# ldyken53/gaussian-splatting-wgpu

Measured on AMD Instinct MI355X. Metric: frames/sec, higher is better.
Workload: dtype f32; 1 GPU; bicycle-like synthetic 6.1M gaussians @1920x1080; gaussians=6100000, width=1920, height=1080, tile_size=16, parallelism=single GPU, visible=2430918, processed=15909895, block_evaluated=6068168, sort_passes=1, depth_ordered_emission=True, tight_binning=True, blend_mode=fused, camera=64-step orbit, moved every frame

## Files before the change

### gaussian-splatting-wgpu_amd/csrc/gs_kernels.h

```cpp
#pragma once
#include "gs_device.h"

void gs_launch_repack(const void* d_aos, uint32_t n, const GsScene& s, hipStream_t st);
void gs_launch_ply_chunk(const void* d_raw, uint32_t m, uint32_t first, const GsPlyTable& t, const GsScene& s, hipStream_t st);
struct GsPreprocessLaunch {
    const void* func;
    uint32_t blocks;
    GsScene s; GsUniforms u; GsFrame f;
    void* gdata; uint32_t* counts; GsTightOut to;
    void* args[6];
};
void gs_preprocess_prepare(GsPreprocessLaunch& L, const GsScene& s, const GsUniforms& u, const GsFrame& f, void* gdata, uint32_t* counts,
                           bool tight, uint32_t* arena, uint32_t* rowptr, GsControl* ctl, uint32_t tight_nb = 0);
void gs_launch_preprocess(GsPreprocessLaunch& L, hipStream_t st);
void gs_launch_zero(void* p, uint64_t bytes, hipStream_t st);
uint32_t gs_scan_blocks(uint32_t n);
void gs_launch_scan(const uint32_t* counts, uint32_t n, uint32_t* offsets, unsigned long long* status, uint32_t* ticket, GsControl* ctl,
                    hipStream_t st);
uint64_t gs_emit_chunks(uint64_t capacity);
void gs_launch_emit_balanced(const void* gdata, const void* grec, const uint32_t* chunk_table, const GsFrame& f, uint32_t* keys, uint32_t* values,
                             GsControl* ctl, uint32_t grid, uint32_t hist_bits, uint32_t hist_passes, bool keys16, hipStream_t st);
void gs_launch_emit(const void* gdata, const uint32_t* counts, const uint32_t* offsets, const uint32_t* perm, const uint32_t* n_dev,
                    const GsFrame& f, uint32_t* keys, uint32_t* values, GsControl* ctl, hipStream_t st);
void gs_launch_ranges16(const uint16_t* tiles, const GsControl* ctl, uint32_t capacity, uint32_t T, uint32_t* ranges, uint32_t grid,
                        uint32_t* sticky, GsReport* rep, hipStream_t st);
void gs_launch_rebuild_keys(const uint16_t* tiles, const uint32_t* vals, const uint32_t* counts, uint32_t count, uint32_t n, uint32_t id_mask,
                            uint32_t* keys, hipStream_t st);
void gs_launch_ranges(const uint32_t* keys, const GsControl* ctl, uint32_t capacity, uint32_t T, uint32_t* ranges, uint32_t grid,
                      uint32_t* sticky, GsReport* rep, hipStream_t st);
uint32_t gs_sort_tiles(uint64_t capacity);
void gs_launch_sort(uint32_t* keysA, uint32_t* valsA, uint32_t* keysB, uint32_t* valsB, GsControl* ctl, uint32_t* tickets, uint32_t* hist,
                    const uint32_t* n_ptr, uint32_t capacity, uint32_t passes, uint32_t bits, uint32_t by_tile, uint32_t* status,
                    uint32_t grid, bool have_hist, const uint32_t* aux_table, uint32_t* aux_out, hipStream_t st, uint32_t** out_keys,
                    uint32_t** out_vals, bool keys16 = false);
int gs_launch_blend(const void* gdata, const uint32_t* values, const uint32_t* ranges, const GsFrame& f, uint32_t* rgba8, float* rgbf,
                    bool aux, float* alpha, float* depth, GsControl* ctl, uint32_t* tile_depth, bool exact, uint32_t ablation, bool masked, hipStream_t st, uint32_t* prof = nullptr,
                    uint32_t* prof_blocks = nullptr);
void gs_launch_debug_view(const uint32_t* ranges, const GsFrame& f, uint32_t view, uint32_t* rgba8, hipStream_t st);
void gs_launch_assemble(const void* slabs, void* image, uint32_t width, uint32_t height, const uint32_t* d_px_bounds, uint32_t n_slabs,
                        uint64_t slab_stride_px, hipStream_t st);
uint32_t gs_gsort_tiles(uint32_t n);
uint64_t gs_gsort_scratch_bytes(uint32_t n);
void gs_launch_gsort(const uint32_t* words, const uint32_t* aux_in, uint32_t n, void* scratch, void* grec, uint32_t* chunk_table, uint32_t chunk_cap,
                     uint32_t* tot_visible, uint32_t* tot_quantity, uint32_t grid, hipStream_t st);
uint32_t gs_rows_sort_tiles(uint64_t row_cap);
uint32_t gs_rows_chunks(uint64_t row_cap);
void gs_launch_rows(const uint32_t* arena, const void* grec, const uint32_t* chunk_table, uint32_t* rows_sorted, GsControl* ctl, uint32_t* sort_status, uint32_t row_cap,
                    uint32_t* M3, uint32_t* tileoff, uint32_t* rowtot, const GsFrame& f, uint32_t* values, uint32_t* ranges, uint32_t cus,
                    uint32_t* sticky, GsReport* rep, hipStream_t st, void (*mark)(void*, int), void* mark_arg);
void gs_launch_rows_rebuild_keys(const uint32_t* ranges, uint32_t T, const uint32_t* vals, const uint32_t* counts, uint32_t count, uint32_t n,
                                 uint32_t* keys, hipStream_t st);
void gs_launch_pick(const void* gdata, const uint32_t* values, const uint32_t* ranges, const GsFrame& f, uint32_t id_mask, const void* d_queries,
                    uint32_t n, void* d_results, uint32_t max_contrib, void* d_contrib, hipStream_t st);
```

### gaussian-splatting-wgpu_amd/csrc/gs_runtime.hip

```cpp
#include <hip/hip_runtime.h>

#include <algorithm>
#include <cmath>
#include <cstdarg>
#include <cstddef>
#include <cstdio>
#include <cstring>
#include <mutex>
#include <new>
#include <vector>

#include "../../include/gsplat/gs_abi.h"
#include "gs_kernels.h"
#include "gs_tight.h"

#define GS_EXPORT extern "C" __attribute__((visibility("default")))

static thread_local char g_err[512] = "";
static int32_t fail(int32_t code, const char* fmt, ...) {
    va_list ap;
    va_start(ap, fmt);
    vsnprintf(g_err, sizeof(g_err), fmt, ap);
    va_end(ap);
    return code;
}
#define HIP_TRY(expr)                                                                                       \
    do {                                                                                                    \
        hipError_t e_ = (expr);                                                                             \
        if (e_ != hipSuccess)                                                                               \
            return fail(e_ == hipErrorOutOfMemory ? GS_ERR_OUT_OF_MEMORY : GS_ERR_HIP, "%s: %s", #expr,      \
                        hipGetErrorString(e_));                                                             \
    } while (0)

#include <dlfcn.h>
namespace {
struct Roctx {
    int (*push)(const char*) = nullptr;
    int (*pop)() = nullptr;
    Roctx() {
// ... 9 lines not shown
Roctx& roctx() { static Roctx r; return r; }
const char* const kStageRange[] = {"gsplat:process_gaussians", "gsplat:exclusive_scan", "gsplat:write_tile_ids", "gsplat:radix_sort",
                                   "gsplat:compute_ranges", "gsplat:compute_tiles"};
}

#define GS_EV_RING 256
struct gs_ctx {
    gs_config cfg{};
    hipStream_t stream = nullptr;
    bool own_stream = false;
    GsFrame frame{};
    uint32_t T = 0, passes = 0, key_bits = 0;
    uint32_t tile_passes = 0, tile_bits = 0;
    bool tile16 = false;
    bool last_keys16 = false;
    uint32_t* keysG = nullptr;
    bool keysG_valid = false;
    int emit_order = 2;
    bool index_order = true;
    uint32_t debug_view = 0;
    uint32_t fif = 1;
    std::vector<gs_ctx*> shadows;
    bool is_shadow = false;
    gs_ctx* last = nullptr;
    uint32_t rr = 0;
    uint64_t cap_hint = 0, row_hint = 0;
    hipEvent_t ev_done = nullptr;
    uint64_t next_ticket = 1;
    struct { uint64_t ticket; gs_ctx* member; } tickets[64] = {};
    std::mutex ticket_mu;
    bool tile_cull = true;
    bool last_tight = false;
    uint32_t grid_persist = 0;
    uint32_t blend_ablation = 0;
    uint32_t* blend_prof = nullptr;
    uint32_t blend_prof_blocks = 0;
    void* scene_mem = nullptr;
    size_t scene_bytes = 0;
    GsScene scene{};
    uint32_t n = 0;
    uint32_t* counts = nullptr;
    uint32_t* offsets = nullptr;
    void* gdata = nullptr;
    uint64_t capacity = 0;
    uint32_t *keysA = nullptr, *valsA = nullptr, *keysB = nullptr, *valsB = nullptr;
    uint32_t *keysU = nullptr, *valsU = nullptr;
    uint32_t* chunk_table = nullptr;
    uint32_t *keysS = nullptr, *valsS = nullptr;
    void* ctl_mem = nullptr;
    size_t ctl_bytes = 0;
    GsControl* ctl = nullptr;
    unsigned long long* scan_status = nullptr;
    uint32_t* tile_depth = nullptr;
    uint32_t* sort_status = nullptr;
    uint32_t* rows_status = nullptr;
    void* grec = nullptr;
    uint32_t tight_nb = 0;
    void* gsort_scratch = nullptr;
    uint64_t row_cap = 0;
    uint32_t *arena = nullptr, *rows_sorted = nullptr, *rowptr = nullptr;
    uint32_t *M3 = nullptr, *tileoff = nullptr, *rowtot = nullptr;
    bool tight_ok = false;
    bool scene_borrowed = false;
    uint32_t last_passes = 0;
    bool last_by_index = true;
    uint32_t blend_walkers = 1;
// ... 105 lines not shown
    if (cfg->device < 0 || cfg->device >= ndev) return fail(GS_ERR_INVALID_ARGUMENT, "gs_create: device %d of %d", cfg->device, ndev);
    HIP_TRY(hipSetDevice(cfg->device));

    gs_ctx* c = new (std::nothrow) gs_ctx();
    if (!c) return fail(GS_ERR_OUT_OF_MEMORY, "gs_create: host allocation failed");
    c->cfg = *cfg;
    GsFrame& f = c->frame;
    f.width = cfg->width; f.height = cfg->height; f.tile_size = cfg->tile_size;
    f.ntx = tiles_f32(cfg->width, cfg->tile_size);
    f.nty = tiles_f32(cfg->height, cfg->tile_size);
    if (f.ntx >= 32768 || f.nty >= 65536) { delete c; return fail(GS_ERR_INVALID_ARGUMENT, "gs_create: canvas too large"); }
    f.col0 = cfg->col_begin;
    f.col1 = cfg->col_end;
    if (f.col0 == 0 && f.col1 == 0) f.col1 = f.ntx;
    if (f.col1 > f.ntx || f.col0 >= f.col1) { delete c; return fail(GS_ERR_INVALID_ARGUMENT, "gs_create: bad tile-column slab [%u,%u) of %u", f.col0, f.col1, f.ntx); }
    f.full = (f.col0 == 0 && f.col1 == f.ntx) ? 1u : 0u;
    f.px0 = f.col0 * f.tile_size;
    f.slab_w = std::min(f.width, f.col1 * f.tile_size) - f.px0;
    c->T = f.ntx * f.nty;
    const uint64_t max_key = ((uint64_t)f.nty * f.ntx + f.ntx) * 1000ull + 999ull;
    if (max_key > 0xFFFFFFFFull) { delete c; return fail(GS_ERR_INVALID_ARGUMENT, "gs_create: tile ids overflow the 32-bit key (write_tile_ids.wgsl:29)"); }
    c->key_bits = bits_for(max_key);
    c->passes = (c->key_bits + 7) / 8;
    const uint32_t tbits = bits_for((uint64_t)f.nty * f.ntx + f.ntx);
    c->tile_passes = (tbits + 7) / 8;
    c->tile_bits = (tbits + c->tile_passes - 1) / c->tile_passes;
    c->tile16 = ((uint64_t)f.nty * f.ntx + f.ntx) < 0xFFFFull;
    if ((uint64_t)(f.ntx + 1) * (f.nty + 1) > GS_COUNT_MASK) { delete c; return fail(GS_ERR_INVALID_ARGUMENT, "gs_create: canvas has too many tiles"); }
    c->tight_ok = f.ntx <= 255u && f.nty <= 255u;

    hipDeviceProp_t prop;
    HIP_TRY(hipGetDeviceProperties(&prop, cfg->device));
    c->grid_persist = (uint32_t)prop.multiProcessorCount * 4;
    if (cfg->stream) c->stream = (hipStream_t)cfg->stream;
    else { HIP_TRY(hipStreamCreateWithFlags(&c->stream, hipStreamNonBlocking)); c->own_stream = true; }

    HIP_TRY(hipMalloc((void**)&c->ranges, (size_t)c->T * 4));
    HIP_TRY(hipMemset(c->ranges, 0, (size_t)c->T * 4));
    const size_t px = (size_t)f.slab_w * f.height;
    HIP_TRY(hipMalloc((void**)&c->rgba8, px * 4));
    HIP_TRY(hipMemset(c->rgba8, 0, px * 4));
    if (cfg->flags & GS_FLAG_F32_TAP) HIP_TRY(hipMalloc((void**)&c->rgbf, px * 12));
    if (cfg->flags & GS_FLAG_AUX_OUTPUTS) {
        HIP_TRY(hipMalloc((void**)&c->alpha, px * 4));
        HIP_TRY(hipMalloc((void**)&c->depth, px * 4));
        HIP_TRY(hipMemset(c->alpha, 0, px * 4));
        HIP_TRY(hipMemset(c->depth, 0, px * 4));
    }
    HIP_TRY(hipHostMalloc((void**)&c->h_ctl, sizeof(GsControl), hipHostMallocDefault));
    memset(c->h_ctl, 0, sizeof(GsControl));
    HIP_TRY(hipMalloc((void**)&c->d_pxb, 65 * 4));
    HIP_TRY(hipMalloc((void**)&c->tileoff, 256 * 256 * 4));
    HIP_TRY(hipMalloc((void**)&c->rowtot, 256 * 4));
    HIP_TRY(hipMalloc((void**)&c->sticky, 4 * 4));
    HIP_TRY(hipMemset(c->sticky, 0, 4 * 4));
    HIP_TRY(hipHostMalloc((void**)&c->h_rep, sizeof(GsReport), hipHostMallocDefault));
    memset(c->h_rep, 0, sizeof(GsReport));
    if (cfg->flags & GS_FLAG_TIMING) {
        for (auto& row : c->ev)
            for (auto& e : row) HIP_TRY(hipEventCreate(&e));
        c->have_events = true;
    }
    c->fif = (c->own_stream && f.full) ? 3u : 1u;
    *out = c;
    return GS_OK;
}
// ... 128 lines not shown
    hipFree(d);
    return rc;
}

static inline void mark(gs_ctx* c, int i) {
    if (!c->have_events) return;
    hipEventRecord(c->ev[c->frames % GS_EV_RING][i], c->stream);
    Roctx& r = roctx();
    if (r.push) {
        if (i > 0) r.pop();
        if (i < GS_STAGE_COUNT) r.push(kStageRange[i]);
    }
}

static void mark_cb(void* p, int i) { mark((gs_ctx*)p, i); }

static int32_t record_frame(gs_ctx* c, const GsUniforms& u, bool debug, void* ext_rgba8, bool tight) {
    const GsFrame& f = c->frame;
    hipStream_t st = c->stream;
    gs_launch_zero(c->ctl_mem, tight ? c->ctl_bytes_tight : c->ctl_bytes, st);
    c->h_ctl_valid = false;
    if (debug) HIP_TRY(hipMemsetAsync(c->gdata, 0, std::max<size_t>((size_t)c->n * 64, 256), st));
    mark(c, 0);
    gs_preprocess_prepare(c->pre, c->scene, u, f, c->gdata, c->counts, tight, c->arena, c->rowptr, c->ctl, c->tight_nb);
    gs_launch_preprocess(c->pre, st);
    mark(c, 1);
    const bool by_index = !tight && (debug || c->index_order);
    bool keys16 = false;
    if (tight) {
        gs_launch_gsort(c->counts, c->rowptr, c->n, c->gsort_scratch, c->grec, c->chunk_table, (uint32_t)gs_emit_chunks(std::max(c->capacity, c->row_cap)),
                        &c->ctl->num_visible, &c->ctl->num_slots, c->grid_persist, st);
        mark(c, 2);
        gs_launch_rows(c->arena, c->grec, c->chunk_table, c->rows_sorted, c->ctl, c->rows_status, (uint32_t)c->row_cap, c->M3, c->tileoff, c->rowtot, f, c->valsA,
                       c->ranges, c->grid_persist / 4u, c->sticky, c->h_rep, st, mark_cb, c);
        c->keysS = nullptr;
        c->valsS = c->valsA;
        mark(c, 4);
    } else if (by_index) {
        gs_launch_scan(c->counts, c->n, c->offsets, c->scan_status, &c->ctl->scan_ticket[0], c->ctl, st);
        mark(c, 2);
        gs_launch_emit(c->gdata, c->counts, c->offsets, nullptr, nullptr, f, c->keysA, c->valsA, c->ctl, st);
    } else {
        gs_launch_gsort(c->counts, nullptr, c->n, c->gsort_scratch, c->grec, c->chunk_table, (uint32_t)gs_emit_chunks(std::max(c->capacity, c->row_cap)),
                        &c->ctl->num_visible, &c->ctl->num_intersections, c->grid_persist, st);
        mark(c, 2);
        gs_launch_emit_balanced(c->gdata, c->grec, c->chunk_table, f, c->keysA, c->valsA, c->ctl, c->grid_persist * 2,
                                c->tile_bits, c->tile_passes, c->tile16, st);
        keys16 = c->tile16;
    }
    if (debug) {
        if (!c->keysU) {
            HIP_TRY(hipMalloc((void**)&c->keysU, (size_t)c->capacity * 4));
            HIP_TRY(hipMalloc((void**)&c->valsU, (size_t)c->capacity * 4));
        }
        HIP_TRY(hipMemcpyAsync(c->keysU, c->keysA, (size_t)c->capacity * 4, hipMemcpyDeviceToDevice, st));
        HIP_TRY(hipMemcpyAsync(c->valsU, c->valsA, (size_t)c->capacity * 4, hipMemcpyDeviceToDevice, st));
    }
    if (!tight) {
        mark(c, 3);
        if (by_index)
            gs_launch_sort(c->keysA, c->valsA, c->keysB, c->valsB, c->ctl, c->ctl->sort_ticket, &c->ctl->hist[0][0], &c->ctl->num_intersections,
                           (uint32_t)c->capacity, c->passes, 8, 0, c->sort_status, c->grid_persist, false, nullptr, nullptr, st, &c->keysS, &c->valsS);
        else
            gs_launch_sort(c->keysA, c->valsA, c->keysB, c->valsB, c->ctl, c->ctl->sort_ticket, &c->ctl->hist[0][0], &c->ctl->num_intersections,
                           (uint32_t)c->capacity, c->tile_passes, c->tile_bits, keys16 ? 0 : 1, c->sort_status, c->grid_persist, true,
                           nullptr, nullptr, st, &c->keysS, &c->valsS, keys16);
        mark(c, 4);
// ... 156 lines not shown
}

static gs_ctx* last_of(gs_ctx* c) { return (c && c->last) ? c->last : c; }

GS_EXPORT int32_t gs_wait(gs_ctx* c) {
    if (!c) return fail(GS_ERR_INVALID_ARGUMENT, "gs_wait: null ctx");
    int32_t first = wait_one(c);
    char msg[sizeof(g_err)];
    if (first != GS_OK) memcpy(msg, g_err, sizeof(msg));
    for (gs_ctx* s : c->shadows) {
        const int32_t rc = wait_one(s);
        if (rc != GS_OK && first == GS_OK) { first = rc; memcpy(msg, g_err, sizeof(msg)); }
    }
    c->cap_hint = std::max(c->cap_hint, c->capacity);
    c->row_hint = std::max(c->row_hint, c->row_cap);
    for (gs_ctx* s : c->shadows) { c->cap_hint = std::max(c->cap_hint, s->capacity); c->row_hint = std::max(c->row_hint, s->row_cap); }
    if (first != GS_OK) memcpy(g_err, msg, sizeof(msg));
    return first;
}

static int32_t set_option_one(gs_ctx* c, int32_t key, int64_t value);
static int32_t add_shadow(gs_ctx* c) {
    gs_config cfg = c->cfg;
    cfg.stream = nullptr;
    cfg.max_intersections = 0;
    gs_ctx* s = nullptr;
    int32_t rc = gs_create(&cfg, &s);
    if (rc != GS_OK) return rc;
    s->fif = 1;
    s->is_shadow = true;
    rc = gs_share_splats(s, c);
    if (rc != GS_OK) { gs_destroy(s); return rc; }
    s->emit_order = c->emit_order; s->tile_cull = c->tile_cull; s->debug_view = c->debug_view;
    s->blend_ablation = c->blend_ablation; s->grid_persist = c->grid_persist; s->timed_from = 0; s->tight_nb = c->tight_nb;
    s->use_graph = c->use_graph;
    c->shadows.push_back(s);
    return GS_OK;
}

GS_EXPORT int32_t gs_render(gs_ctx* c, const void* uniforms) {
    if (!c || !uniforms) return fail(GS_ERR_INVALID_ARGUMENT, "gs_render: null argument");
    gs_ctx* t = c;
    if (c->fif > 1 && c->scene_mem) {
        if (c->pending && c->shadows.size() + 1 < c->fif) {
            int32_t rc = add_shadow(c);
            if (rc != GS_OK) return rc;
            c->rr = (uint32_t)c->shadows.size();
        }
        if (!c->shadows.empty()) {
            const uint32_t slot = c->rr++ % (uint32_t)(c->shadows.size() + 1);
            t = slot ? c->shadows[slot - 1] : c;
        }
        if (t->capacity < c->cap_hint || t->row_cap < c->row_hint) {
            HIP_TRY(hipSetDevice(t->cfg.device));
            if (t->pending) { int32_t rc = wait_one(t); if (rc != GS_OK && rc != GS_ERR_TRUNCATED) return rc; }
            hipFree(t->keysU); hipFree(t->valsU); t->keysU = t->valsU = nullptr;
            int32_t rc = alloc_kv(t, std::max(t->capacity, c->cap_hint), std::max(t->row_cap, c->row_hint));
            if (rc != GS_OK) return rc;
            t->have_frame = false;
        }
    }
    const int32_t rc = render_common(t, uniforms, false, nullptr);
    if (rc == GS_OK) c->last = t;
    return rc;
}
GS_EXPORT int32_t gs_render_host(gs_ctx* c, const void* uniforms, void* host_dst, uint64_t size, uint64_t* ticket) {
    if (!c || !uniforms || !host_dst || !ticket) return fail(GS_ERR_INVALID_ARGUMENT, "gs_render_host: null argument");
// ... 633 lines not shown
```

### gaussian-splatting-wgpu_amd/csrc/k_rows.hip

```cpp
#include "gs_device.h"
#include "gs_tight.h"

typedef uint32_t gs_item3 __attribute__((ext_vector_type(3), aligned(4)));

#ifndef RA_ITEMS
#define RA_ITEMS 8
#endif
#ifndef RA_WAVES
#define RA_WAVES 8
#endif
#define RA_THREADS (RA_WAVES * 64)
#define RA_TILE (RA_THREADS * RA_ITEMS)
#define RA_AGG (1u << 30)
#define RA_PREFIX (2u << 30)
#define RA_FLAGS (3u << 30)
#define RA_VALUE (~RA_FLAGS)

#ifndef RB_CH
#define RB_CH 512u
#endif
#define RB_IT (RB_CH / 256u)
#ifndef RB_SB
#define RB_SB 2048u
#endif
// ... 170 lines not shown
            const uint32_t r = (j & 1) ? (rank2[j >> 1] >> 16) : (rank2[j >> 1] & 0xFFFFu);
            const uint32_t pos = sh.hist[w][d] + r;
            sh.u.it[pos * 3 + 0] = ix[j];
            sh.u.it[pos * 3 + 1] = iy[j];
            sh.u.it[pos * 3 + 2] = iz[j];
        }
        __syncthreads();
        const uint32_t nvalid = sh.nvalid;
#pragma unroll
        for (int j = 0; j < RA_ITEMS; ++j) {
            const uint32_t pos = j * RA_THREADS + tid;
            if (pos < nvalid) {
                gs_item3 v;
                v.x = sh.u.it[pos * 3 + 0]; v.y = sh.u.it[pos * 3 + 1]; v.z = sh.u.it[pos * 3 + 2];
                const uint32_t g = sh.gbase[v.y & 0xFFu] + pos;
                if (g < row_cap) *reinterpret_cast<gs_item3*>(rows_out + (uint64_t)g * 3u) = v;
            }
        }
        __syncthreads();
    }
}

__device__ __forceinline__ unsigned long long wave_incl_scan64(unsigned long long v, uint32_t lane) {
#pragma unroll
    for (int d = 1; d < 64; d <<= 1) {
        const uint32_t lo = __shfl_up((uint32_t)v, d, 64), hi = __shfl_up((uint32_t)(v >> 32), d, 64);
        if ((int)lane >= d) v += ((unsigned long long)hi << 32) | lo;
    }
    return v;
}
struct RowTables {
    uint32_t ibase[257];
    uint32_t cbase[257];
    uint32_t w4[8];
};
__device__ __forceinline__ void row_tables(RowTables& T, const GsControl* ctl, uint32_t row_cap, uint32_t tid) {
    const uint32_t lane = tid & 63, w = tid >> 6;
    const bool on = tid < 256u;
    const uint32_t c = on ? gs_rowhist(ctl, tid) : 0u;
    const unsigned long long ic = wave_incl_scan64(c, lane);
    if (on && lane == 63) { T.w4[w] = (uint32_t)(ic > 0xFFFFFFFFull ? 0xFFFFFFFFull : ic); }
    __syncthreads();
    uint32_t i0 = 0, cc = 0;
    if (on) {
        unsigned long long b = ic - c;
        for (uint32_t k = 0; k < w; ++k) b += T.w4[k];
        const unsigned long long e = b + c;
        i0 = b > row_cap ? row_cap : (uint32_t)b;
        const uint32_t i1 = e > row_cap ? row_cap : (uint32_t)e;
        cc = i1 - i0;
        T.ibase[tid] = i0;
        if (tid == 255u) T.ibase[256] = i1;
    }
    const uint32_t ch = (cc + RB_CH - 1u) / RB_CH;
    const uint32_t ih = wave_incl_scan(ch, lane);
    if (on && lane == 63) T.w4[4 + w] = ih;
    __syncthreads();
    if (on) {
        uint32_t bh = 0;
        for (uint32_t k = 0; k < w; ++k) bh += T.w4[4 + k];
        T.cbase[tid] = bh + ih - ch;
        if (tid == 255u) T.cbase[256] = bh + ih;
    }
    __syncthreads();
}
__device__ __forceinline__ uint32_t row_of_chunk(const RowTables& T, uint32_t c) {
    const uint32_t lane = threadIdx.x & 63u;
    uint32_t v[4];
#pragma unroll
    for (int k = 0; k < 4; ++k) v[k] = T.cbase[lane + 64u * k];
    uint32_t r = 0;
#pragma unroll
    for (int k = 0; k < 4; ++k) r += (uint32_t)__popcll(__ballot(v[k] <= c && (lane + 64u * k) != 0u));
    return r;
}

__global__ __launch_bounds__(256) void gs_rows_count_kernel(const uint32_t* __restrict__ rows, const GsControl* ctl, uint32_t* __restrict__ M3,
                                                            uint32_t chunk_cap, uint32_t row_cap) {
    __shared__ RowTables T;
    __shared__ int s_diff[257];
    __shared__ uint32_t s_w[4];
    const uint32_t tid = threadIdx.x, lane = tid & 63, w = tid >> 6;
    row_tables(T, ctl, row_cap, tid);
    uint32_t nch = T.cbase[256];
    if (nch > chunk_cap) nch = chunk_cap;
    for (uint32_t c = blockIdx.x; c < nch; c += gridDim.x) {
        const uint32_t r = row_of_chunk(T, c);
        const uint32_t i0 = T.ibase[r] + (c - T.cbase[r]) * RB_CH;
        const uint32_t i1 = (i0 + RB_CH < T.ibase[r + 1]) ? i0 + RB_CH : T.ibase[r + 1];
        s_diff[tid] = 0;
        if (tid == 0) s_diff[256] = 0;
        __syncthreads();
#pragma unroll
        for (int k = 0; k < (int)(RB_CH / 256u); ++k) {
            const uint32_t i = i0 + k * 256u + tid;
            if (i < i1) {
                const uint32_t w1 = rows[(uint64_t)i * 3u + 1u];
                const uint32_t tlo = (w1 >> 8) & 0xFFu, len = ((w1 >> 16) & 0xFFu) + 1u;
                atomicAdd(&s_diff[tlo], 1);
                atomicAdd(&s_diff[tlo + len > 256u ? 256u : tlo + len], -1);
            }
        }
        __syncthreads();
        const uint32_t v = (uint32_t)s_diff[tid];
        const uint32_t incl = wave_incl_scan(v, lane);
        if (lane == 63) s_w[w] = incl;
        __syncthreads();
        uint32_t b = 0;
        for (uint32_t k = 0; k < w; ++k) b += s_w[k];
        M3[(uint64_t)c * 256u + tid] = b + incl;
        __syncthreads();
    }
}

__global__ __launch_bounds__(1024) void gs_rows_scan_kernel(const GsControl* ctl, uint32_t* __restrict__ M3, uint32_t* __restrict__ tileoff,
                                                            uint32_t* __restrict__ rowtot, uint32_t chunk_cap, uint32_t row_cap) {
    __shared__ RowTables T;
    __shared__ unsigned long long s_part[4][256];
    __shared__ unsigned long long s_ex[256];
    __shared__ unsigned long long s_w[4];
    const uint32_t tid = threadIdx.x, c = tid & 255u, p = tid >> 8, r = blockIdx.x;
    row_tables(T, ctl, row_cap, tid);
    uint32_t c0 = T.cbase[r], c1 = T.cbase[r + 1];
    if (c0 > chunk_cap) c0 = chunk_cap;
    if (c1 > chunk_cap) c1 = chunk_cap;
    const uint32_t nch = c1 - c0, per = (nch + 3u) / 4u;
    const uint32_t j0 = c0 + (p * per < nch ? p * per : nch), j1 = c0 + ((p + 1u) * per < nch ? (p + 1u) * per : nch);
    unsigned long long sum = 0;
    for (uint32_t j = j0; j < j1; j += 8u) {
        uint32_t v[8];
#pragma unroll
        for (int k = 0; k < 8; ++k) v[k] = (j + k < j1) ? M3[(uint64_t)(j + k) * 256u + c] : 0u;
#pragma unroll
        for (int k = 0; k < 8; ++k) sum += v[k];
    }
    s_part[p][c] = sum;
    __syncthreads();
    unsigned long long run = 0, tot = 0;
#pragma unroll
    for (int k = 0; k < 4; ++k) { const unsigned long long t = s_part[k][c]; if (k < (int)p) run += t; tot += t; }
    for (uint32_t j = j0; j < j1; j += 8u) {
        uint32_t v[8];
#pragma unroll
        for (int k = 0; k < 8; ++k) v[k] = (j + k < j1) ? M3[(uint64_t)(j + k) * 256u + c] : 0u;
#pragma unroll
        for (int k = 0; k < 8; ++k) {
            if (j + k < j1) M3[(uint64_t)(j + k) * 256u + c] = run > 0xFFFFFFFFull ? 0xFFFFFFFFu : (uint32_t)run;
            run += v[k];
        }
    }
    if (p == 0) {
        const uint32_t lane = tid & 63, w = tid >> 6;
        unsigned long long incl = tot;
#pragma unroll
        for (int d = 1; d < 64; d <<= 1) {
            const uint32_t lo = __shfl_up((uint32_t)incl, d, 64), hi = __shfl_up((uint32_t)(incl >> 32), d, 64);
// ... 2 lines not shown
        if (lane == 63) s_w[w] = incl;
        s_ex[c] = incl - tot;
    }
    __syncthreads();
    if (p == 0) {
        const uint32_t w = tid >> 6;
        unsigned long long b = 0, all = 0;
#pragma unroll
        for (int k = 0; k < 4; ++k) { if (k < (int)w) b += s_w[k]; all += s_w[k]; }
        const unsigned long long ex = b + s_ex[c];
        tileoff[r * 256u + c] = ex > 0xFFFFFFFFull ? 0xFFFFFFFFu : (uint32_t)ex;
        if (c == 0) rowtot[r] = all > 0xFFFFFFFFull ? 0xFFFFFFFFu : (uint32_t)all;
    }
}

struct ExpandShared {
    RowTables T;
    uint32_t rbase[257];
    uint32_t w0[RB_CH], w1[RB_CH], w2[RB_CH];
    uint32_t hist[4][256];
    uint32_t gbase[256];
    uint32_t wsum[8];
    uint32_t nvalid, total;
    unsigned char cols[RB_SB];
    union {
        struct { uint32_t P[RB_CH + 1]; unsigned short mark[RB_SB]; } e;
        uint32_t vals[RB_SB];
    } x;
};

__global__ __launch_bounds__(256) void gs_rows_expand_kernel(const uint32_t* __restrict__ rows, GsControl* ctl, const uint32_t* __restrict__ M3,
                                                             const uint32_t* __restrict__ tileoff, const uint32_t* __restrict__ rowtot, GsFrame f,
                                                             uint32_t* __restrict__ values, uint32_t* __restrict__ ranges, uint32_t chunk_cap,
                                                             uint32_t row_cap, uint32_t* sticky, GsReport* rep) {
    __shared__ ExpandShared S;
    const uint32_t tid = threadIdx.x, lane = tid & 63, w = tid >> 6;
    const unsigned long long lt_mask = (1ull << lane) - 1ull;
    const uint32_t ns = f.tile_size >= 16u ? 2u : 1u;
    const uint32_t hole = f.ntx < 128u ? 127u : 255u;
    const int nbits = f.ntx < 128u ? 7 : 8;
    row_tables(S.T, ctl, row_cap, tid);
    {
        const uint32_t v = tid < f.nty ? rowtot[tid] : 0u;
        unsigned long long incl = v;
#pragma unroll
        for (int d = 1; d < 64; d <<= 1) {
            const uint32_t lo = __shfl_up((uint32_t)incl, d, 64), hi = __shfl_up((uint32_t)(incl >> 32), d, 64);
            if ((int)lane >= d) incl += ((unsigned long long)hi << 32) | lo;
        }
        __shared__ unsigned long long s_r[4];
        if (lane == 63) s_r[w] = incl;
        __syncthreads();
        unsigned long long b = 0;
        for (uint32_t k = 0; k < w; ++k) b += s_r[k];
        const unsigned long long ex = b + incl - v;
        S.rbase[tid] = ex > 0xFFFFFFFFull ? 0xFFFFFFFFu : (uint32_t)ex;
        if (tid == 255u) S.rbase[256] = (b + incl) > 0xFFFFFFFFull ? 0xFFFFFFFFu : (uint32_t)(b + incl);
        __syncthreads();
    }
    if (blockIdx.x == 0 && tid == 0) {
        const uint32_t I = S.rbase[256];
        ctl->num_intersections = I;
        ctl->num_items = S.T.ibase[256];
        if (I > f.capacity) ctl->overflow = 1u;
        gs_frame_report(ctl, I, S.T.ibase[256], f.capacity, sticky, rep);
    }
    for (uint32_t r = blockIdx.x; r < f.nty; r += gridDim.x) {
        if (tid < f.ntx) {
            const uint32_t endoff = (tid + 1u < 256u) ? tileoff[r * 256u + tid + 1u] : rowtot[r];
            const unsigned long long e = (unsigned long long)S.rbase[r] + endoff;
            ranges[r * f.ntx + tid] = e > 0xFFFFFFFFull ? 0xFFFFFFFFu : (uint32_t)e;
        }
    }
    uint32_t nch = S.T.cbase[256];
    if (nch > chunk_cap) nch = chunk_cap;
    gs_item3 nit[RB_IT];
    uint32_t n_r = 0, n_ni = 0, n_tstart = 0, n_done = 0;
    auto prefetch = [&](uint32_t c) {
        n_r = row_of_chunk(S.T, c);
        const uint32_t i0 = S.T.ibase[n_r] + (c - S.T.cbase[n_r]) * RB_CH;
        const uint32_t i1 = (i0 + RB_CH < S.T.ibase[n_r + 1]) ? i0 + RB_CH : S.T.ibase[n_r + 1];
        n_ni = i1 - i0;
#pragma unroll
        for (int k = 0; k < (int)RB_IT; ++k) {
            const uint32_t e = tid * RB_IT + k;
            nit[k] = *reinterpret_cast<const gs_item3*>(rows + (uint64_t)(i0 + (e < n_ni ? e : 0u)) * 3u);
        }
        n_tstart = S.rbase[n_r] + tileoff[n_r * 256u + tid];
        n_done = M3[(uint64_t)c * 256u + tid];
    };
    if (blockIdx.x < nch) prefetch(blockIdx.x);
    for (uint32_t c = blockIdx.x; c < nch; c += gridDim.x) {
        const uint32_t ni = n_ni;
        uint32_t len[RB_IT], lsum = 0;
#pragma unroll
        for (int k = 0; k < (int)RB_IT; ++k) {
            const uint32_t e = tid * RB_IT + k;
            len[k] = 0u;
            if (e < ni) {
                S.w0[e] = nit[k].x; S.w1[e] = nit[k].y; S.w2[e] = nit[k].z;
                len[k] = ((nit[k].y >> 16) & 0xFFu) + 1u;
            }
            lsum += len[k];
        }
        const uint32_t tstart = n_tstart;
        uint32_t done = n_done;
        if (c + gridDim.x < nch) prefetch(c + gridDim.x);
        {
            const uint32_t incl = wave_incl_scan(lsum, lane);
            if (lane == 63) S.wsum[w] = incl;
            __syncthreads();
            uint32_t b = 0, all = 0;
#pragma unroll
            for (int k = 0; k < 4; ++k) { if (k < (int)w) b += S.wsum[k]; all += S.wsum[k]; }
            uint32_t run = b + incl - lsum;
#pragma unroll
            for (int k = 0; k < (int)RB_IT; ++k) { S.x.e.P[tid * RB_IT + k] = run; run += len[k]; }
            if (tid == 0) { S.x.e.P[RB_CH] = all; S.total = all; }
        }
        __syncthreads();
        const uint32_t ninst = S.total;
        for (uint32_t s0 = 0; s0 < ninst; s0 += RB_SB) {
            if (s0) {
                __syncthreads();
                uint32_t l2[RB_IT], ls = 0;
#pragma unroll
                for (int k = 0; k < (int)RB_IT; ++k) { const uint32_t e = tid * RB_IT + k; l2[k] = e < ni ? ((S.w1[e] >> 16) & 0xFFu) + 1u : 0u; ls += l2[k]; }
                const uint32_t incl = wave_incl_scan(ls, lane);
                if (lane == 63) S.wsum[w] = incl;
                __syncthreads();
                uint32_t b = 0;
#pragma unroll
                for (int k = 0; k < 4; ++k) if (k < (int)w) b += S.wsum[k];
                uint32_t run = b + incl - ls;
#pragma unroll
                for (int k = 0; k < (int)RB_IT; ++k) { S.x.e.P[tid * RB_IT + k] = run; run += l2[k]; }
                if (tid == 0) S.x.e.P[RB_CH] = ninst;
            }
            for (uint32_t k = tid; k < RB_SB / 2u; k += 256u) reinterpret_cast<uint32_t*>(S.x.e.mark)[k] = 0u;
            for (uint32_t k = lane; k < 256; k += 64) S.hist[w][k] = 0u;
// ... 102 lines not shown
#pragma unroll
            for (int j = 0; j < (int)RB_PER; ++j) {
                const uint32_t pos = j * 256u + tid;
                if (pos < nvalid) {
                    const uint32_t dst = S.gbase[S.cols[pos]] + pos;
                    if (dst < f.capacity) values[dst] = S.x.vals[pos];
                }
            }
        }
        __syncthreads();
    }
}

__global__ __launch_bounds__(256) void gs_rows_rebuild_keys_kernel(const uint32_t* __restrict__ ranges, uint32_t T, const uint32_t* __restrict__ vals,
                                                                   const uint32_t* __restrict__ counts, uint32_t count, uint32_t n,
                                                                   uint32_t* __restrict__ keys) {
    for (uint32_t i = blockIdx.x * 256u + threadIdx.x; i < count; i += gridDim.x * 256u) {
        uint32_t lo = 0, hi = T;
        while (lo < hi) {
            const uint32_t mid = (lo + hi) >> 1;
            if (ranges[mid] > i) hi = mid; else lo = mid + 1u;
        }
        const uint32_t g = vals[i] & GS_ID_MASK;
        keys[i] = lo * 1000u + (g < n ? counts[g] >> GS_COUNT_BITS : 0u);
    }
}

#ifndef RB_CNT_WG
#define RB_CNT_WG 8u
#endif
#ifndef RB_EXP_WG
#define RB_EXP_WG 6u
#endif
uint32_t gs_rows_sort_tiles(uint64_t row_cap) { return (uint32_t)((row_cap + RA_TILE - 1) / RA_TILE); }
uint32_t gs_rows_chunks(uint64_t row_cap) { return (uint32_t)(row_cap / RB_CH + 256u); }
void gs_launch_rows(const uint32_t* arena, const void* grec, const uint32_t* chunk_table, uint32_t* rows_sorted, GsControl* ctl, uint32_t* sort_status, uint32_t row_cap,
                    uint32_t* M3, uint32_t* tileoff, uint32_t* rowtot, const GsFrame& f, uint32_t* values, uint32_t* ranges, uint32_t cus,
                    uint32_t* sticky, GsReport* rep, hipStream_t st, void (*mark)(void*, int), void* mark_arg) {
    const uint32_t chunk_cap = gs_rows_chunks(row_cap);
    if (!cus) cus = 1;
    hipLaunchKernelGGL(gs_rows_sort_kernel, dim3(cus * 3u), dim3(RA_THREADS), 0, st, arena, (const uint4*)grec, chunk_table, rows_sorted, ctl, sort_status,
                       row_cap, f.nty);
    if (mark) mark(mark_arg, 3);
    hipLaunchKernelGGL(gs_rows_count_kernel, dim3(cus * RB_CNT_WG), dim3(256), 0, st, (const uint32_t*)rows_sorted, (const GsControl*)ctl, M3, chunk_cap, row_cap);
    hipLaunchKernelGGL(gs_rows_scan_kernel, dim3(f.nty), dim3(1024), 0, st, (const GsControl*)ctl, M3, tileoff, rowtot, chunk_cap, row_cap);
    hipLaunchKernelGGL(gs_rows_expand_kernel, dim3(cus * RB_EXP_WG), dim3(256), 0, st, (const uint32_t*)rows_sorted, ctl, (const uint32_t*)M3,
                       (const uint32_t*)tileoff, (const uint32_t*)rowtot, f, values, ranges, chunk_cap, row_cap, sticky, rep);
}
void gs_launch_rows_rebuild_keys(const uint32_t* ranges, uint32_t T, const uint32_t* vals, const uint32_t* counts, uint32_t count, uint32_t n,
                                 uint32_t* keys, hipStream_t st) {
    if (!count) return;
    const uint32_t blocks = (count + 255u) / 256u;
    hipLaunchKernelGGL(gs_rows_rebuild_keys_kernel, dim3(blocks < 4096u ? blocks : 4096u), dim3(256), 0, st, ranges, T, vals, counts, count, n, keys);
}
```

Baseline: 1378 frames/s.

## Group row chunks into multi-chunk runs for count/scan/expand

Adds a run abstraction in the rows binning pipeline: consecutive chunks within a row are grouped into runs of K chunks, sized so the total run count is close to a target (by default a multiple of the expand grid). The count kernel now builds one histogram per run, so M3 stores per-run prefix counts. The scan works over runs and the expand kernel walks K chunks of a run in sequence, reloading tile start and done counts only at run heads. The aim is fewer M3 entries, less scan work and fewer per-chunk global reads. The cost is coarser load balance and longer serial work per block.

Result: no change. 1391 frames/s, median of 6 (+1.0%).

```diff
diff --git a/gaussian-splatting-wgpu_amd/csrc/gs_kernels.h b/gaussian-splatting-wgpu_amd/csrc/gs_kernels.h
--- a/gaussian-splatting-wgpu_amd/csrc/gs_kernels.h
+++ b/gaussian-splatting-wgpu_amd/csrc/gs_kernels.h
@@ -47,7 +47,7 @@
 uint32_t gs_rows_chunks(uint64_t row_cap);
 void gs_launch_rows(const uint32_t* arena, const void* grec, const uint32_t* chunk_table, uint32_t* rows_sorted, GsControl* ctl, uint32_t* sort_status, uint32_t row_cap,
                     uint32_t* M3, uint32_t* tileoff, uint32_t* rowtot, const GsFrame& f, uint32_t* values, uint32_t* ranges, uint32_t cus,
-                    uint32_t* sticky, GsReport* rep, hipStream_t st, void (*mark)(void*, int), void* mark_arg);
+                    uint32_t runs, uint32_t* sticky, GsReport* rep, hipStream_t st, void (*mark)(void*, int), void* mark_arg);
 void gs_launch_rows_rebuild_keys(const uint32_t* ranges, uint32_t T, const uint32_t* vals, const uint32_t* counts, uint32_t count, uint32_t n,
                                  uint32_t* keys, hipStream_t st);
 void gs_launch_pick(const void* gdata, const uint32_t* values, const uint32_t* ranges, const GsFrame& f, uint32_t id_mask, const void* d_queries,
diff --git a/gaussian-splatting-wgpu_amd/csrc/gs_runtime.hip b/gaussian-splatting-wgpu_amd/csrc/gs_runtime.hip
--- a/gaussian-splatting-wgpu_amd/csrc/gs_runtime.hip
+++ b/gaussian-splatting-wgpu_amd/csrc/gs_runtime.hip
@@ -5,6 +5,7 @@
 #include <cstdarg>
 #include <cstddef>
 #include <cstdio>
+#include <cstdlib>
 #include <cstring>
 #include <mutex>
 #include <new>
@@ -80,6 +81,7 @@
     bool tile_cull = true;
     bool last_tight = false;
     uint32_t grid_persist = 0;
+    uint32_t rows_runs = 0;
     uint32_t blend_ablation = 0;
     uint32_t* blend_prof = nullptr;
     uint32_t blend_prof_blocks = 0;
@@ -251,6 +253,10 @@
     hipDeviceProp_t prop;
     HIP_TRY(hipGetDeviceProperties(&prop, cfg->device));
     c->grid_persist = (uint32_t)prop.multiProcessorCount * 4;
+    if (const char* e = getenv("GSPLAT_ROWS_RUNS")) {
+        const unsigned long long v = strtoull(e, nullptr, 10);
+        c->rows_runs = v > 0x7FFFFFFFull ? 0x7FFFFFFFu : (uint32_t)v;
+    }
     if (cfg->stream) c->stream = (hipStream_t)cfg->stream;
     else { HIP_TRY(hipStreamCreateWithFlags(&c->stream, hipStreamNonBlocking)); c->own_stream = true; }
 
@@ -445,7 +451,7 @@
                         &c->ctl->num_visible, &c->ctl->num_slots, c->grid_persist, st);
         mark(c, 2);
         gs_launch_rows(c->arena, c->grec, c->chunk_table, c->rows_sorted, c->ctl, c->rows_status, (uint32_t)c->row_cap, c->M3, c->tileoff, c->rowtot, f, c->valsA,
-                       c->ranges, c->grid_persist / 4u, c->sticky, c->h_rep, st, mark_cb, c);
+                       c->ranges, c->grid_persist / 4u, c->rows_runs, c->sticky, c->h_rep, st, mark_cb, c);
         c->keysS = nullptr;
         c->valsS = c->valsA;
         mark(c, 4);
@@ -668,7 +674,7 @@
     rc = gs_share_splats(s, c);
     if (rc != GS_OK) { gs_destroy(s); return rc; }
     s->emit_order = c->emit_order; s->tile_cull = c->tile_cull; s->debug_view = c->debug_view;
-    s->blend_ablation = c->blend_ablation; s->grid_persist = c->grid_persist; s->timed_from = 0; s->tight_nb = c->tight_nb;
+    s->blend_ablation = c->blend_ablation; s->grid_persist = c->grid_persist; s->rows_runs = c->rows_runs; s->timed_from = 0; s->tight_nb = c->tight_nb;
     s->use_graph = c->use_graph;
     c->shadows.push_back(s);
     return GS_OK;
diff --git a/gaussian-splatting-wgpu_amd/csrc/k_rows.hip b/gaussian-splatting-wgpu_amd/csrc/k_rows.hip
--- a/gaussian-splatting-wgpu_amd/csrc/k_rows.hip
+++ b/gaussian-splatting-wgpu_amd/csrc/k_rows.hip
@@ -226,9 +226,11 @@
 struct RowTables {
     uint32_t ibase[257];
     uint32_t cbase[257];
+    uint32_t ubase[257];
+    uint32_t K;
     uint32_t w4[8];
 };
-__device__ __forceinline__ void row_tables(RowTables& T, const GsControl* ctl, uint32_t row_cap, uint32_t tid) {
+__device__ __forceinline__ void row_tables(RowTables& T, const GsControl* ctl, uint32_t row_cap, uint32_t G, uint32_t tid) {
     const uint32_t lane = tid & 63, w = tid >> 6;
     const bool on = tid < 256u;
     const uint32_t c = on ? gs_rowhist(ctl, tid) : 0u;
@@ -257,6 +259,20 @@
         if (tid == 255u) T.cbase[256] = bh + ih;
     }
     __syncthreads();
+    const uint32_t nch = T.cbase[256], g = G ? G : 1u;
+    uint32_t K = nch / g + (nch % g ? 1u : 0u);
+    if (K < 1u) K = 1u;
+    const uint32_t ru = ch / K + (ch % K ? 1u : 0u);
+    const uint32_t iu = wave_incl_scan(ru, lane);
+    if (on && lane == 63) T.w4[w] = iu;
+    __syncthreads();
+    if (on) {
+        uint32_t bu = 0;
+        for (uint32_t k = 0; k < w; ++k) bu += T.w4[k];
+        T.ubase[tid] = bu + iu - ru;
+        if (tid == 255u) { T.ubase[256] = bu + iu; T.K = K; }
+    }
+    __syncthreads();
 }
 __device__ __forceinline__ uint32_t row_of_chunk(const RowTables& T, uint32_t c) {
     const uint32_t lane = threadIdx.x & 63u;
@@ -268,31 +284,49 @@
     for (int k = 0; k < 4; ++k) r += (uint32_t)__popcll(__ballot(v[k] <= c && (lane + 64u * k) != 0u));
     return r;
 }
+__device__ __forceinline__ uint32_t row_of_run(const RowTables& T, uint32_t u) {
+    const uint32_t lane = threadIdx.x & 63u;
+    uint32_t v[4];
+#pragma unroll
+    for (int k = 0; k < 4; ++k) v[k] = T.ubase[lane + 64u * k];
+    uint32_t r = 0;
+#pragma unroll
+    for (int k = 0; k < 4; ++k) r += (uint32_t)__popcll(__ballot(v[k] <= u && (lane + 64u * k) != 0u));
+    return r;
+}
 
 __global__ __launch_bounds__(256) void gs_rows_count_kernel(const uint32_t* __restrict__ rows, const GsControl* ctl, uint32_t* __restrict__ M3,
-                                                            uint32_t chunk_cap, uint32_t row_cap) {
+                                                            uint32_t chunk_cap, uint32_t row_cap, uint32_t G) {
     __shared__ RowTables T;
     __shared__ int s_diff[257];
     __shared__ uint32_t s_w[4];
     const uint32_t tid = threadIdx.x, lane = tid & 63, w = tid >> 6;
-    row_tables(T, ctl, row_cap, tid);
-    uint32_t nch = T.cbase[256];
-    if (nch > chunk_cap) nch = chunk_cap;
-    for (uint32_t c = blockIdx.x; c < nch; c += gridDim.x) {
-        const uint32_t r = row_of_chunk(T, c);
-        const uint32_t i0 = T.ibase[r] + (c - T.cbase[r]) * RB_CH;
-        const uint32_t i1 = (i0 + RB_CH < T.ibase[r + 1]) ? i0 + RB_CH : T.ibase[r + 1];
+    row_tables(T, ctl, row_cap, G, tid);
+    uint32_t nrun = T.ubase[256];
+    if (nrun > chunk_cap) nrun = chunk_cap;
+    const uint32_t K = T.K;
+    for (uint32_t u = blockIdx.x; u < nrun; u += gridDim.x) {
+        const uint32_t r = row_of_run(T, u);
+        const uint32_t i0 = T.ibase[r] + (u - T.ubase[r]) * K * RB_CH;
+        const uint32_t left = T.ibase[r + 1] - i0;
+        const uint32_t ni = (unsigned long long)K * RB_CH < left ? K * RB_CH : left;
         s_diff[tid] = 0;
         if (tid == 0) s_diff[256] = 0;
         __syncthreads();
-#pragma unroll
-        for (int k = 0; k < (int)(RB_CH / 256u); ++k) {
-            const uint32_t i = i0 + k * 256u + tid;
-            if (i < i1) {
-                const uint32_t w1 = rows[(uint64_t)i * 3u + 1u];
-                const uint32_t tlo = (w1 >> 8) & 0xFFu, len = ((w1 >> 16) & 0xFFu) + 1u;
-                atomicAdd(&s_diff[tlo], 1);
-                atomicAdd(&s_diff[tlo + len > 256u ? 256u : tlo + len], -1);
+        for (uint32_t o = 0; o < ni; o += 4u * 256u) {
+            uint32_t w1[4];
+#pragma unroll
+            for (int k = 0; k < 4; ++k) {
+                const uint32_t i = o + k * 256u + tid;
+                w1[k] = rows[(uint64_t)(i0 + (i < ni ? i : 0u)) * 3u + 1u];
+            }
+#pragma unroll
+            for (int k = 0; k < 4; ++k) {
+                if (o + k * 256u + tid < ni) {
+                    const uint32_t tlo = (w1[k] >> 8) & 0xFFu, len = ((w1[k] >> 16) & 0xFFu) + 1u;
+                    atomicAdd(&s_diff[tlo], 1);
+                    atomicAdd(&s_diff[tlo + len > 256u ? 256u : tlo + len], -1);
+                }
             }
         }
         __syncthreads();
@@ -302,20 +336,20 @@
         __syncthreads();
         uint32_t b = 0;
         for (uint32_t k = 0; k < w; ++k) b += s_w[k];
-        M3[(uint64_t)c * 256u + tid] = b + incl;
+        M3[(uint64_t)u * 256u + tid] = b + incl;
         __syncthreads();
     }
 }
 
 __global__ __launch_bounds__(1024) void gs_rows_scan_kernel(const GsControl* ctl, uint32_t* __restrict__ M3, uint32_t* __restrict__ tileoff,
-                                                            uint32_t* __restrict__ rowtot, uint32_t chunk_cap, uint32_t row_cap) {
+                                                            uint32_t* __restrict__ rowtot, uint32_t chunk_cap, uint32_t row_cap, uint32_t G) {
     __shared__ RowTables T;
     __shared__ unsigned long long s_part[4][256];
     __shared__ unsigned long long s_ex[256];
     __shared__ unsigned long long s_w[4];
     const uint32_t tid = threadIdx.x, c = tid & 255u, p = tid >> 8, r = blockIdx.x;
-    row_tables(T, ctl, row_cap, tid);
-    uint32_t c0 = T.cbase[r], c1 = T.cbase[r + 1];
+    row_tables(T, ctl, row_cap, G, tid);
+    uint32_t c0 = T.ubase[r], c1 = T.ubase[r + 1];
     if (c0 > chunk_cap) c0 = chunk_cap;
     if (c1 > chunk_cap) c1 = chunk_cap;
     const uint32_t nch = c1 - c0, per = (nch + 3u) / 4u;
@@ -384,14 +418,14 @@
 __global__ __launch_bounds__(256) void gs_rows_expand_kernel(const uint32_t* __restrict__ rows, GsControl* ctl, const uint32_t* __restrict__ M3,
                                                              const uint32_t* __restrict__ tileoff, const uint32_t* __restrict__ rowtot, GsFrame f,
                                                              uint32_t* __restrict__ values, uint32_t* __restrict__ ranges, uint32_t chunk_cap,
-                                                             uint32_t row_cap, uint32_t* sticky, GsReport* rep) {
+                                                             uint32_t row_cap, uint32_t G, uint32_t* sticky, GsReport* rep) {
     __shared__ ExpandShared S;
     const uint32_t tid = threadIdx.x, lane = tid & 63, w = tid >> 6;
     const unsigned long long lt_mask = (1ull << lane) - 1ull;
     const uint32_t ns = f.tile_size >= 16u ? 2u : 1u;
     const uint32_t hole = f.ntx < 128u ? 127u : 255u;
     const int nbits = f.ntx < 128u ? 7 : 8;
-    row_tables(S.T, ctl, row_cap, tid);
+    row_tables(S.T, ctl, row_cap, G, tid);
     {
         const uint32_t v = tid < f.nty ? rowtot[tid] : 0u;
         unsigned long long incl = v;
@@ -424,25 +458,40 @@
             ranges[r * f.ntx + tid] = e > 0xFFFFFFFFull ? 0xFFFFFFFFu : (uint32_t)e;
         }
     }
-    uint32_t nch = S.T.cbase[256];
-    if (nch > chunk_cap) nch = chunk_cap;
+    uint32_t nrun = S.T.ubase[256];
+    if (nrun > chunk_cap) nrun = chunk_cap;
+    const uint32_t K = S.T.K;
     gs_item3 nit[RB_IT];
-    uint32_t n_r = 0, n_ni = 0, n_tstart = 0, n_done = 0;
-    auto prefetch = [&](uint32_t c) {
-        n_r = row_of_chunk(S.T, c);
-        const uint32_t i0 = S.T.ibase[n_r] + (c - S.T.cbase[n_r]) * RB_CH;
-        const uint32_t i1 = (i0 + RB_CH < S.T.ibase[n_r + 1]) ? i0 + RB_CH : S.T.ibase[n_r + 1];
-        n_ni = i1 - i0;
+    uint32_t n_ni = 0, n_tstart = 0, n_done = 0;
+    bool n_head = false;
+    uint32_t q_u = blockIdx.x - gridDim.x, q_k = 0, q_nk = 0, q_i = 0, q_iend = 0;
+    auto prefetch = [&]() -> bool {
+        n_head = q_k == q_nk;
+        if (n_head) {
+            q_u += gridDim.x;
+            if (q_u >= nrun) return false;
+            const uint32_t r = row_of_run(S.T, q_u);
+            const uint32_t j = q_u - (uint32_t)__builtin_amdgcn_readfirstlane((int)S.T.ubase[r]);
+            const uint32_t left = (uint32_t)__builtin_amdgcn_readfirstlane((int)(S.T.cbase[r + 1] - S.T.cbase[r])) - j * K;
+            q_nk = left < K ? left : K;
+            q_k = 0;
+            q_i = (uint32_t)__builtin_amdgcn_readfirstlane((int)S.T.ibase[r]) + j * K * RB_CH;
+            q_iend = (uint32_t)__builtin_amdgcn_readfirstlane((int)S.T.ibase[r + 1]);
+            n_tstart = S.rbase[r] + tileoff[r * 256u + tid];
+            n_done = M3[(uint64_t)q_u * 256u + tid];
+        }
+        n_ni = q_iend - q_i < RB_CH ? q_iend - q_i : RB_CH;
 #pragma unroll
         for (int k = 0; k < (int)RB_IT; ++k) {
             const uint32_t e = tid * RB_IT + k;
-            nit[k] = *reinterpret_cast<const gs_item3*>(rows + (uint64_t)(i0 + (e < n_ni ? e : 0u)) * 3u);
-        }
-        n_tstart = S.rbase[n_r] + tileoff[n_r * 256u + tid];
-        n_done = M3[(uint64_t)c * 256u + tid];
+            nit[k] = *reinterpret_cast<const gs_item3*>(rows + (uint64_t)(q_i + (e < n_ni ? e : 0u)) * 3u);
+        }
+        q_i += n_ni;
+        ++q_k;
+        return true;
     };
-    if (blockIdx.x < nch) prefetch(blockIdx.x);
-    for (uint32_t c = blockIdx.x; c < nch; c += gridDim.x) {
+    uint32_t tstart = 0, done = 0;
+    for (bool more = prefetch(); more;) {
         const uint32_t ni = n_ni;
         uint32_t len[RB_IT], lsum = 0;
 #pragma unroll
@@ -455,9 +504,11 @@
             }
             lsum += len[k];
         }
-        const uint32_t tstart = n_tstart;
-        uint32_t done = n_done;
-        if (c + gridDim.x < nch) prefetch(c + gridDim.x);
+        if (n_head) {
+            tstart = n_tstart;
+            done = n_done;
+        }
+        more = prefetch();
         {
             const uint32_t incl = wave_incl_scan(lsum, lane);
             if (lane == 63) S.wsum[w] = incl;
@@ -626,20 +677,24 @@
 #ifndef RB_EXP_WG
 #define RB_EXP_WG 6u
 #endif
+#ifndef RB_RUNS
+#define RB_RUNS 2u
+#endif
 uint32_t gs_rows_sort_tiles(uint64_t row_cap) { return (uint32_t)((row_cap + RA_TILE - 1) / RA_TILE); }
 uint32_t gs_rows_chunks(uint64_t row_cap) { return (uint32_t)(row_cap / RB_CH + 256u); }
 void gs_launch_rows(const uint32_t* arena, const void* grec, const uint32_t* chunk_table, uint32_t* rows_sorted, GsControl* ctl, uint32_t* sort_status, uint32_t row_cap,
                     uint32_t* M3, uint32_t* tileoff, uint32_t* rowtot, const GsFrame& f, uint32_t* values, uint32_t* ranges, uint32_t cus,
-                    uint32_t* sticky, GsReport* rep, hipStream_t st, void (*mark)(void*, int), void* mark_arg) {
+                    uint32_t runs, uint32_t* sticky, GsReport* rep, hipStream_t st, void (*mark)(void*, int), void* mark_arg) {
     const uint32_t chunk_cap = gs_rows_chunks(row_cap);
     if (!cus) cus = 1;
+    if (!runs) runs = cus * RB_EXP_WG * RB_RUNS;
     hipLaunchKernelGGL(gs_rows_sort_kernel, dim3(cus * 3u), dim3(RA_THREADS), 0, st, arena, (const uint4*)grec, chunk_table, rows_sorted, ctl, sort_status,
                        row_cap, f.nty);
     if (mark) mark(mark_arg, 3);
-    hipLaunchKernelGGL(gs_rows_count_kernel, dim3(cus * RB_CNT_WG), dim3(256), 0, st, (const uint32_t*)rows_sorted, (const GsControl*)ctl, M3, chunk_cap, row_cap);
-    hipLaunchKernelGGL(gs_rows_scan_kernel, dim3(f.nty), dim3(1024), 0, st, (const GsControl*)ctl, M3, tileoff, rowtot, chunk_cap, row_cap);
+    hipLaunchKernelGGL(gs_rows_count_kernel, dim3(cus * RB_CNT_WG), dim3(256), 0, st, (const uint32_t*)rows_sorted, (const GsControl*)ctl, M3, chunk_cap, row_cap, runs);
+    hipLaunchKernelGGL(gs_rows_scan_kernel, dim3(f.nty), dim3(1024), 0, st, (const GsControl*)ctl, M3, tileoff, rowtot, chunk_cap, row_cap, runs);
     hipLaunchKernelGGL(gs_rows_expand_kernel, dim3(cus * RB_EXP_WG), dim3(256), 0, st, (const uint32_t*)rows_sorted, ctl, (const uint32_t*)M3,
-                       (const uint32_t*)tileoff, (const uint32_t*)rowtot, f, values, ranges, chunk_cap, row_cap, sticky, rep);
+                       (const uint32_t*)tileoff, (const uint32_t*)rowtot, f, values, ranges, chunk_cap, row_cap, runs, sticky, rep);
 }
 void gs_launch_rows_rebuild_keys(const uint32_t* ranges, uint32_t T, const uint32_t* vals, const uint32_t* counts, uint32_t count, uint32_t n,
                                  uint32_t* keys, hipStream_t st) {
```
